# xiph/rav1e

Hardware: AMD Instinct MI355X
Metric: RDO-candidate Mpixels/s (dist+fwd_tx+mc) at 4K speed-6 (higher is better)
Workload: dtype u8

## Files before the change

rav1e_amd/csrc/cand_common.hpp:

```cpp
#pragma once
#include <type_traits>

#include "common.hpp"
#include "dist_common.hpp"
#include "mc_common.hpp"

namespace r1cand {

#include "mc_taps_packed.inc"

template <int CTRL>
__device__ __forceinline__ int32_t dpp(int32_t x) {
  return __builtin_amdgcn_update_dpp(0, x, CTRL, 0xf, 0xf, true);
}
template <int CTRL>
__device__ __forceinline__ int32_t bfly_lanes(int32_t x, int32_t sm) {
  return __mul24(x, sm | 1) + dpp<CTRL>(x);
}
struct LaneSigns { int32_t s1, s2; };
template <int TS>
__device__ __forceinline__ LaneSigns lane_signs(int lane) {
  LaneSigns s;
  if constexpr (TS == 8) {
    s.s1 = -(int32_t)((lane ^ (lane >> 2)) & 1);
    s.s2 = -(int32_t)(((lane >> 1) ^ (lane >> 2)) & 1);
  } else {
    s.s1 = -(int32_t)(lane & 1);
    s.s2 = 0;
  }
  return s;
}
template <int TS>
__device__ __forceinline__ uint32_t habs_lanes(int32_t x, LaneSigns sg) {
  x = bfly_lanes<0xB1>(x, sg.s1);
  if constexpr (TS == 8) x = bfly_lanes<0x4E>(x, sg.s2);
  const int32_t ax = iabs32(x);
  const int32_t ap = TS == 8 ? dpp<0x141>(ax) : dpp<0x4E>(ax);
  return (uint32_t)(ax > ap ? ax : ap);
}

__device__ __forceinline__ uint32_t sad_u32(uint32_t a, uint32_t b, uint32_t acc) {
  uint32_t r;
  asm("v_sad_u32 %0, %1, %2, %3" : "=v"(r) : "v"(a), "v"(b), "v"(acc));
  return r;
}

typedef short v2s_t __attribute__((ext_vector_type(2)));
typedef unsigned short v2us_t __attribute__((ext_vector_type(2)));
__device__ __forceinline__ uint32_t pk_add(uint32_t a, uint32_t b) {
  return __builtin_bit_cast(uint32_t, (v2s_t)(__builtin_bit_cast(v2s_t, a) + __builtin_bit_cast(v2s_t, b)));
}
__device__ __forceinline__ uint32_t pk_sub(uint32_t a, uint32_t b) {
  return __builtin_bit_cast(uint32_t, (v2s_t)(__builtin_bit_cast(v2s_t, a) - __builtin_bit_cast(v2s_t, b)));
}
__device__ __forceinline__ uint32_t pk_mad(uint32_t x, uint32_t s, uint32_t p) {
  uint32_t r;
  asm("v_pk_mad_i16 %0, %1, %2, %3" : "=v"(r) : "v"(x), "v"(s), "v"(p));
  return r;
}
__device__ __forceinline__ uint32_t pk_max(uint32_t a, uint32_t b) {
  uint32_t r;
  asm("v_pk_max_i16 %0, %1, %2" : "=v"(r) : "v"(a), "v"(b));
  return r;
}
__device__ __forceinline__ uint32_t pk_min(uint32_t a, uint32_t b) {
  uint32_t r;
  asm("v_pk_min_i16 %0, %1, %2" : "=v"(r) : "v"(a), "v"(b));
  return r;
}
__device__ __forceinline__ uint32_t pk_pair(int32_t lo, int32_t hi) {
  return __builtin_amdgcn_perm((uint32_t)hi, (uint32_t)lo, 0x05040100u);
}
__device__ __forceinline__ void pk_bfly8_s2(const uint32_t (&a)[8], uint32_t (&d)[8]) {
  uint32_t b[8];
#pragma unroll
  for (int k = 0; k < 4; k++) {
    b[2 * k] = pk_add(a[2 * k], a[2 * k + 1]);
    b[2 * k + 1] = pk_sub(a[2 * k], a[2 * k + 1]);
  }
  d[0] = pk_add(b[0], b[2]); d[2] = pk_sub(b[0], b[2]);
  d[1] = pk_add(b[1], b[3]); d[3] = pk_sub(b[1], b[3]);
  d[4] = pk_add(b[4], b[6]); d[6] = pk_sub(b[4], b[6]);
  d[5] = pk_add(b[5], b[7]); d[7] = pk_sub(b[5], b[7]);
}
__device__ __forceinline__ uint32_t habs_lanes_pk(uint32_t x, uint32_t m1, uint32_t m2, uint32_t acc) {
  x = pk_mad(x, m1, (uint32_t)dpp<0xB1>((int32_t)x));
  x = pk_mad(x, m2, (uint32_t)dpp<0x4E>((int32_t)x));
  const uint32_t ax = pk_max(x, pk_sub(0u, x));
  const uint32_t mx = pk_max(ax, (uint32_t)dpp<0x141>((int32_t)ax));
  return __builtin_amdgcn_udot2(__builtin_bit_cast(v2us_t, mx), __builtin_bit_cast(v2us_t, 0x00010001u),
                                acc, false);
}

__device__ __forceinline__ uint32_t ashr_pair(int32_t lo, int32_t hi, int sh) {
  return __builtin_amdgcn_perm((uint32_t)(hi >> sh), (uint32_t)(lo >> sh), 0x05040100u);
}

__device__ __forceinline__ int32_t dot2_seed0(uint32_t a, uint32_t b) {
  int32_t r;
  asm("v_dot2_i32_i16 %0, %1, %2, 0" : "=v"(r) : "v"(a), "v"(b));
  return r;
}
__device__ __forceinline__ int32_t dot2_seed64(uint32_t a, uint32_t b) {
  int32_t r;
  asm("v_dot2_i32_i16 %0, %1, %2, 64" : "=v"(r) : "v"(a), "v"(b));
  return r;
}
__device__ __forceinline__ int32_t dot2_seed(uint32_t a, uint32_t b, int32_t c_uniform) {
  int32_t r;
  asm("v_dot2_i32_i16 %0, %1, %2, %3" : "=v"(r) : "v"(a), "v"(b), "s"(c_uniform));
  return r;
}
__device__ __forceinline__ int32_t dot4_seed(uint32_t a, uint32_t b, int32_t c_uniform) {
  int32_t r;
  asm("v_dot4_i32_i8 %0, %1, %2, %3" : "=v"(r) : "v"(a), "v"(b), "s"(c_uniform));
  return r;
}

template <int BPP> struct Taps;
template <> struct Taps<1> { uint32_t fx0, fx1, ty[4]; };
template <> struct Taps<2> { uint32_t tx[4], ty[4]; };
template <int BPP, int W, int H>
__device__ __forceinline__ Taps<BPP> load_taps(int cf, int rf, int mx, int my) {
  const int fxi = r1mc::filter_index(mx, W), fyi = r1mc::filter_index(my, H);
  Taps<BPP> t;
  if constexpr (BPP == 1) {
    t.fx0 = kTapI8[fxi][cf][0];
    t.fx1 = kTapI8[fxi][cf][1];
  }
#pragma unroll
  for (int j = 0; j < 4; j++) {
    if constexpr (BPP == 2) t.tx[j] = kTapI16[fxi][cf][j];
    t.ty[j] = kTapI16[fyi][rf][j];
  }
  return t;
}
__device__ __forceinline__ bool taps_six(const Taps<1> &t) {
  return __all(((t.ty[0] & 0xffffu) | (t.ty[3] >> 16)) == 0);
}
__device__ __forceinline__ bool taps_six(const Taps<2> &t) {
  return __all(((t.ty[0] & 0xffffu) | (t.ty[3] >> 16) | (t.tx[0] & 0xffffu) | (t.tx[3] >> 16)) == 0);
}

#define R1_ODD_ROW_TAPS(ty, tz)                                                                   \
  do {                                                                                            \
    tz[0] = ty[0] << 16;                                                                          \
    _Pragma("unroll") for (int j = 1; j < 4; j++) tz[j] = __builtin_amdgcn_alignbit(ty[j], ty[j - 1], 16); \
    tz[4] = ty[3] >> 16;                                                                          \
  } while (0)

template <int W, int H, int WS, bool PREP, bool PACK4 = false>
__device__ __forceinline__ void mc8_column_t(const uint8_t *win, int c, const Taps<1> &tp, int32_t *pred, bool six) {
  const uint32_t fx0 = tp.fx0, fx1 = tp.fx1;
  uint32_t ty[4], tz[5];
#pragma unroll
  for (int j = 0; j < 4; j++) ty[j] = tp.ty[j];
  R1_ODD_ROW_TAPS(ty, tz);
  static_assert(!(PREP && PACK4), "the shift-free pack is stated for put_8tap only");
  constexpr int32_t bias = 8192 + 2 + (PREP ? 0 : 32);
  constexpr int WSD = WS / 4;
  const uint32_t *wrow = (const uint32_t *)win + (c >> 2);
  const uint32_t sh8 = 8u * (uint32_t)(c & 3);
  const uint64_t t64 = (((uint64_t)fx1 << 32) | fx0) << sh8;
  const uint32_t t0 = (uint32_t)t64, t1 = (uint32_t)(t64 >> 32);
  const uint32_t t2 = (uint32_t)(((uint64_t)fx1 << sh8) >> 32);
  auto hacc = [&](int r) -> int32_t {
    const uint32_t d0 = wrow[r * WSD], d1 = wrow[r * WSD + 1], d2 = wrow[r * WSD + 2];
    int32_t acc = dot4_seed(d0, t0, bias);
    acc = __builtin_amdgcn_sdot4((int)d1, (int)t1, acc, false);
    acc = __builtin_amdgcn_sdot4((int)d2, (int)t2, acc, false);
    return acc;
  };
  auto hpair = [&](int r) -> uint32_t {
    if constexpr (PACK4) {
      if (r + 1 < H + 7) return pk_pair(hacc(r), hacc(r + 1)) & 0xfffcfffcu;
      return (uint32_t)hacc(r) & 0xfffffffcu;
    } else {
      if (r + 1 < H + 7) return ashr_pair(hacc(r), hacc(r + 1), 2);
      return (uint32_t)(hacc(r) >> 2);
    }
  };
  auto body = [&](auto six_tag) {
    constexpr bool SIX = decltype(six_tag)::value;
    uint32_t pk[5];
    if constexpr (PACK4) pk[0] = SIX ? ((uint32_t)hacc(1) & 0xfffcu) << 16 : hpair(0);
    else pk[0] = SIX ? (uint32_t)(hacc(1) >> 2) << 16 : hpair(0);
#pragma unroll
    for (int j = 1; j < 4; j++) pk[j] = hpair(2 * j);
#pragma unroll
    for (int j = 0; j < H / 2; j++) {
      if (!SIX || j + 1 < H / 2) pk[4] = hpair(2 * j + 8);
      int32_t a0 = PREP ? dot2_seed64(pk[0], ty[0]) : dot2_seed0(pk[0], ty[0]);
#pragma unroll
      for (int k = 1; k < 4; k++)
        a0 = __builtin_amdgcn_sdot2(__builtin_bit_cast(v2s_t, pk[k]),
                                    __builtin_bit_cast(v2s_t, ty[k]), a0, false);
      int32_t a1;
      if constexpr (SIX) {
        a1 = PREP ? dot2_seed64(pk[1], tz[1]) : dot2_seed0(pk[1], tz[1]);
#pragma unroll
        for (int k = 2; k < 4; k++)
          a1 = __builtin_amdgcn_sdot2(__builtin_bit_cast(v2s_t, pk[k]),
                                      __builtin_bit_cast(v2s_t, tz[k]), a1, false);
      } else {
        a1 = PREP ? dot2_seed64(pk[0], tz[0]) : dot2_seed0(pk[0], tz[0]);
#pragma unroll
        for (int k = 1; k < 5; k++)
          a1 = __builtin_amdgcn_sdot2(__builtin_bit_cast(v2s_t, pk[k]),
                                      __builtin_bit_cast(v2s_t, tz[k]), a1, false);
      }
      if constexpr (PREP) {
        pred[2 * j] = a0 >> 7;
        pred[2 * j + 1] = a1 >> 7;
      } else {
        a0 >>= PACK4 ? 13 : 11;
        a1 >>= PACK4 ? 13 : 11;
        pred[2 * j] = a0 < 0 ? 0 : (a0 > 255 ? 255 : a0);
        pred[2 * j + 1] = a1 < 0 ? 0 : (a1 > 255 ? 255 : a1);
      }
#pragma unroll
      for (int k = 0; k < 4; k++) pk[k] = pk[k + 1];
    }
  };
  if (six) body(std::true_type{});
  else body(std::false_type{});
}

template <int W, int H, int WS, bool PREP>
__device__ __forceinline__ void mc16_column_t(const uint8_t *win, int c, const Taps<2> &tp, int bit_depth,
                                              int32_t *pred, bool six) {
  uint32_t tx[4], ty[4], tz[5];
#pragma unroll
  for (int j = 0; j < 4; j++) {
    tx[j] = tp.tx[j];
    ty[j] = tp.ty[j];
  }
  R1_ODD_ROW_TAPS(ty, tz);
  const int ib = r1mc::intermediate_bits(bit_depth);
  const int hsh = 7 - ib, vsh = 7 + ib;
  const int32_t hbias = (1 << (6 - ib)) + (PREP ? 0 : 64);
  const int32_t maxv = (1 << bit_depth) - 1;
  constexpr int WSD = WS / 4;
  const uint32_t *wrow = (const uint32_t *)win + (c >> 1);
  const bool odd = c & 1;
  uint32_t u[5];
  u[0] = odd ? tx[0] << 16 : tx[0];
#pragma unroll
  for (int j = 1; j < 4; j++) u[j] = odd ? __builtin_amdgcn_alignbit(tx[j], tx[j - 1], 16) : tx[j];
  u[4] = odd ? tx[3] >> 16 : 0u;
  auto body = [&](auto six_tag) {
    constexpr bool SIX = decltype(six_tag)::value;
    auto hacc = [&](int r) -> int32_t {
      const uint32_t *p = wrow + r * WSD;
      int32_t acc = dot2_seed(p[0], u[0], hbias);
#pragma unroll
      for (int j = 1; j < (SIX ? 4 : 5); j++)
        acc = __builtin_amdgcn_sdot2(__builtin_bit_cast(v2s_t, p[j]), __builtin_bit_cast(v2s_t, u[j]), acc, false);
      return acc;
    };
    auto hpair = [&](int r) -> uint32_t {
      if (r + 1 < H + 7) return ashr_pair(hacc(r), hacc(r + 1), hsh);
      return (uint32_t)(hacc(r) >> hsh);
    };
    uint32_t pk[5];
    pk[0] = SIX ? (uint32_t)(hacc(1) >> hsh) << 16 : hpair(0);
#pragma unroll
    for (int j = 1; j < 4; j++) pk[j] = hpair(2 * j);
#pragma unroll
    for (int j = 0; j < H / 2; j++) {
      if (!SIX || j + 1 < H / 2) pk[4] = hpair(2 * j + 8);
      int32_t a0 = PREP ? dot2_seed64(pk[0], ty[0]) : dot2_seed0(pk[0], ty[0]);
#pragma unroll
      for (int k = 1; k < 4; k++)
        a0 = __builtin_amdgcn_sdot2(__builtin_bit_cast(v2s_t, pk[k]), __builtin_bit_cast(v2s_t, ty[k]), a0, false);
      int32_t a1;
      if constexpr (SIX) {
        a1 = PREP ? dot2_seed64(pk[1], tz[1]) : dot2_seed0(pk[1], tz[1]);
#pragma unroll
        for (int k = 2; k < 4; k++)
          a1 = __builtin_amdgcn_sdot2(__builtin_bit_cast(v2s_t, pk[k]), __builtin_bit_cast(v2s_t, tz[k]), a1, false);
      } else {
        a1 = PREP ? dot2_seed64(pk[0], tz[0]) : dot2_seed0(pk[0], tz[0]);
#pragma unroll
        for (int k = 1; k < 5; k++)
          a1 = __builtin_amdgcn_sdot2(__builtin_bit_cast(v2s_t, pk[k]), __builtin_bit_cast(v2s_t, tz[k]), a1, false);
      }
      if constexpr (PREP) {
        pred[2 * j] = (a0 >> 7) - 8192;
        pred[2 * j + 1] = (a1 >> 7) - 8192;
      } else {
        a0 >>= vsh;
        a1 >>= vsh;
        pred[2 * j] = a0 < 0 ? 0 : (a0 > maxv ? maxv : a0);
        pred[2 * j + 1] = a1 < 0 ? 0 : (a1 > maxv ? maxv : a1);
      }
#pragma unroll
      for (int k = 0; k < 4; k++) pk[k] = pk[k + 1];
    }
  };
  if (six) body(std::true_type{});
  else body(std::false_type{});
}

template <int BPP, int W, int H, int WS, bool PREP, bool PACK4 = false>
__device__ __forceinline__ void mc_column_fast(const uint8_t *win, int c, const Taps<BPP> &tp, int bit_depth,
                                               int32_t *pred, bool six) {
  static_assert(!PACK4 || BPP == 1, "8 * mid of 16-bit pixels does not fit i16");
  if constexpr (BPP == 1) mc8_column_t<W, H, WS, PREP, PACK4>(win, c, tp, pred, six);
  else mc16_column_t<W, H, WS, PREP>(win, c, tp, bit_depth, pred, six);
}

__device__ __forceinline__ void satd_rows16_s2(const int32_t *v, uint32_t (&d)[8]) {
  uint32_t a[8];
#pragma unroll
  for (int k = 0; k < 8; k++) a[k] = pk_pair(v[k], v[8 + k]);
  pk_bfly8_s2(a, d);
}
template <int W, int H>
__device__ __forceinline__ void satd_tile_store(const int32_t *v, uint32_t *tcol) {
#pragma unroll
  for (int g = 0; g < H / 16; g++) {
    uint32_t d[8];
    satd_rows16_s2(v + g * 16, d);
#pragma unroll
    for (int k = 0; k < 4; k++) {
      tcol[(g * 8 + 2 * k) * W] = pk_add(d[k], d[k + 4]);
      tcol[(g * 8 + 2 * k + 1) * W] = pk_sub(d[k], d[k + 4]);
    }
  }
}
template <int NI, int P>
__device__ __forceinline__ uint32_t satd_tile_rows(const uint32_t *tile, int c) {
  uint32_t acc = 0;
#pragma unroll
  for (int m = 0; m < NI; m++) {
    const uint4 *p = (const uint4 *)(tile + (c + m * P) * 8);
    const uint4 lo = p[0], hi = p[1];
    const uint32_t x[8] = {lo.x, lo.y, lo.z, lo.w, hi.x, hi.y, hi.z, hi.w};
    uint32_t z[8];
    pk_bfly8_s2(x, z);
#pragma unroll
    for (int k = 0; k < 4; k++) {
      const uint32_t mx = pk_max(pk_max(z[k], z[k + 4]), pk_sub(0u, pk_min(z[k], z[k + 4])));
      acc = __builtin_amdgcn_udot2(__builtin_bit_cast(v2us_t, mx), __builtin_bit_cast(v2us_t, 0x00020002u), acc, false);
    }
  }
  return acc;
}

template <int TS, int H, int BD>
__device__ __forceinline__ uint32_t satd_column(const int32_t *v, int lane) {
  const LaneSigns sg = lane_signs<TS>(lane);
  uint32_t acc = 0;
  if constexpr (TS == 8 && BD <= 10) {
    const uint32_t m1 = (uint32_t)sg.s1 | 0x00010001u, m2 = (uint32_t)sg.s2 | 0x00010001u;
    if constexpr (H == 8) {
      uint32_t a[4];
#pragma unroll
      for (int k = 0; k < 4; k++) a[k] = pk_pair(v[k] + v[k + 4], v[k] - v[k + 4]);
      const uint32_t a0 = pk_add(a[0], a[1]), a1 = pk_sub(a[0], a[1]);
      const uint32_t a2 = pk_add(a[2], a[3]), a3 = pk_sub(a[2], a[3]);
      acc = habs_lanes_pk(pk_add(a0, a2), m1, m2, acc);
      acc = habs_lanes_pk(pk_add(a1, a3), m1, m2, acc);
      acc = habs_lanes_pk(pk_sub(a0, a2), m1, m2, acc);
      acc = habs_lanes_pk(pk_sub(a1, a3), m1, m2, acc);
    } else {
#pragma unroll
      for (int g = 0; g < H / 16; g++) {
        uint32_t d[8];
        satd_rows16_s2(v + g * 16, d);
#pragma unroll
        for (int k = 0; k < 4; k++) {
          acc = habs_lanes_pk(pk_add(d[k], d[k + 4]), m1, m2, acc);
          acc = habs_lanes_pk(pk_sub(d[k], d[k + 4]), m1, m2, acc);
        }
      }
    }
    return acc;
  }
#pragma unroll
  for (int g = 0; g < H / TS; g++) {
    int32_t a[TS];
#pragma unroll
    for (int k = 0; k < TS; k++) a[k] = v[g * TS + k];
    if constexpr (TS == 4) {
      const int32_t a0 = a[0] + a[1], a1 = a[0] - a[1];
      const int32_t a2 = a[2] + a[3], a3 = a[2] - a[3];
      a[0] = a0 + a2; a[1] = a1 + a3; a[2] = a0 - a2; a[3] = a1 - a3;
    } else {
      int32_t b[8], d[8];
#pragma unroll
      for (int k = 0; k < 4; k++) {
        b[2 * k] = a[2 * k] + a[2 * k + 1];
        b[2 * k + 1] = a[2 * k] - a[2 * k + 1];
      }
      d[0] = b[0] + b[2]; d[2] = b[0] - b[2];
      d[1] = b[1] + b[3]; d[3] = b[1] - b[3];
      d[4] = b[4] + b[6]; d[6] = b[4] - b[6];
      d[5] = b[5] + b[7]; d[7] = b[5] - b[7];
#pragma unroll
      for (int k = 0; k < 4; k++) {
        a[k] = d[k] + d[k + 4];
        a[k + 4] = d[k] - d[k + 4];
      }
    }
#pragma unroll
    for (int k = 0; k < TS; k++) acc += habs_lanes<TS>(a[k], sg);
  }
  return acc;
}

}
```

rav1e_amd/csrc/mc_window.hpp:

```cpp
#pragma once

namespace r1mc {

constexpr int window_stride(int w, int bpp) { return (((w + 7) * bpp + 3) >> 2) << 2; }

}
```

rav1e_amd/csrc/rdo_cand_kernel.hpp:

```cpp
#pragma once
#include <cstdlib>
#include <type_traits>

#include "cand_common.hpp"
#include "dist_common.hpp"
#include "intra_pred_common.hpp"
#include "itx_common.hpp"
#include "mc_common.hpp"
#include "quant_common.hpp"
#include "rdo_cand_args.hpp"
#include "tx_common.hpp"

#ifdef R1_PHASE_PROF
static __device__ unsigned long long g_phase[4096][8];
#define R1_PROF(i)                                                          \
  do {                                                                      \
    const unsigned long long t_ = __builtin_readcyclecounter();             \
    if (QM == 0 && threadIdx.x == 0 && (blockIdx.x & 63) == 0 && (blockIdx.x >> 6) < 4096) \
      g_phase[blockIdx.x >> 6][i] = t_ - tprev_;                            \
    tprev_ = t_;                                                            \
  } while (0)
#define R1_PROF_INIT unsigned long long tprev_ = __builtin_readcyclecounter()
#else
#define R1_PROF(i) do {} while (0)
#define R1_PROF_INIT do {} while (0)
#endif

namespace {
using r1tx::T;
using r1cand::sad_u32;

template <int BD, int WL, int HL, typename CT, int QM, bool MT = false, int PS = 0>
__global__ __launch_bounds__(64, rdo_waves_hint(BD, WL, HL, QM, MT)) void k_rdo_cand(
    R1Plane org, R1Plane ref, const R1RdoCand *__restrict__ cands, int n,
    uint32_t *__restrict__ sad_out, uint32_t *__restrict__ satd_out,
    CT *__restrict__ coeffs, void *__restrict__ pred_out, RdoQuantArgs qa,
    typename std::conditional<PS == 1, RdoIntraArgs, RdoNoIntraArgs>::type ia) {
  using PL = RdoCandPlan<BD, WL, HL, QM, MT, PS>;
  constexpr int BPP = PL::BPP, W = PL::W, H = PL::H, P = PL::P, NC = PL::NC, TS = PL::TS, WS = PL::WS, FL = PL::FL, HU = PL::HU;
  constexpr bool INTRA = PL::INTRA, SPLIT_T = PL::SPLIT_T, SRC_LDS = PL::SRC_LDS, SRC_LATE = PL::SRC_LATE,
                 SRC_KEEP = PL::SRC_KEEP, SATD_T = PL::SATD_T, COLSHARE = PL::COLSHARE;
  typedef typename PL::TB TB;
  constexpr int LSTRIDE = PL::LSTRIDE, ISTRIDE = PL::ISTRIDE, QT_STRIDE = PL::QT_STRIDE, SRC_ROW = PL::SRC_ROW,
                SRC_CSTRIDE = PL::SRC_CSTRIDE, SATD_STRIDE = PL::SATD_STRIDE, LDS_WORK = PL::LDS_WORK,
                SRC_OFF = PL::SRC_OFF, TKEEP_OFF = PL::TKEEP_OFF, LDS_BYTES = PL::LDS_BYTES;
  static_assert(!INTRA || LDS_BYTES <= RdoCandPlan<BD, WL, HL, QM, MT, 0>::LDS_BYTES,
                "an intra instantiation's LDS must not exceed its inter twin's");
  constexpr int SH0 = r1tx::fwd_shift_ct(WL, HL, BD, 0), SH1 = r1tx::fwd_shift_ct(WL, HL, BD, 1),
                SH2 = r1tx::fwd_shift_ct(WL, HL, BD, 2);
  constexpr bool COL_FOLD = PL::COL_FOLD;
  static_assert(!COL_FOLD || SH0 > 0, "the column family starts from a pending shift[0]");
  constexpr int SH1C = COL_FOLD ? 0 : SH1;
  constexpr bool HALVE2 = PL::HALVE2, MC_PACK4 = PL::MC_PACK4;
  __shared__ __attribute__((aligned(16))) uint8_t smem[LDS_BYTES];
  T *buf = (T *)smem;
  TB *tbuf = (TB *)smem;
  TB *tkeep = COLSHARE ? (TB *)(smem + TKEEP_OFF) : tbuf;

  R1_PROF_INIT;
  const unsigned wg = xcd_contiguous_wg();
  if ((long long)wg * NC >= (long long)n) return;
  const int lane = threadIdx.x;
  const int cl = lane / P, c = lane % P;
  const int cand_i = (int)wg * NC + cl;
  const long long cand = cand_i;
  constexpr bool UNMASK = !(BD == 8 && WL == 6 && HL == 6);
  const bool live_st = cand_i < n;
  const bool live = UNMASK || live_st;
  const int cl_ld = live_st ? cl : n - 1 - (int)wg * NC;
  const long long cand_ld = live_st ? cand : (long long)n - 1;
  R1RdoCand cd = {};
  R1IntraCand ic = {};
  int eset = 0;
  if constexpr (INTRA) {
    if (live) {
      ic = ia.cands[cand_ld];
      eset = (int)cand_ld / ia.edge_group;
      cd.ox = ia.pos_xy[2 * eset];
      cd.oy = ia.pos_xy[2 * eset + 1];
    }
  } else {
    if (live) cd = (cands + (size_t)wg * NC)[cl_ld];
  }
#ifdef R1_PHASE_PROF
  asm volatile("s_waitcnt vmcnt(0)" ::: "memory");
  R1_PROF(5);
#endif
  constexpr bool QUANT = QM != 0;
  constexpr int PPK = QM == 2 ? (H * BPP + 3) / 4 : 1;
  uint32_t ppk[PPK];
#pragma unroll
  for (int k = 0; k < PPK; k++) ppk[k] = 0;

  T v[H];
#pragma unroll
  for (int r = 0; r < H; r++) v[r] = 0;
  const bool col_live = live && c < W;
  const uint8_t *src_l = smem + SRC_OFF + cl * SRC_CSTRIDE + c * BPP;
  constexpr int CHS = SRC_ROW >= 16 ? 16 : SRC_ROW;
  constexpr int CPR = SRC_ROW / CHS;
  constexpr int RPP = P / CPR;
  constexpr int SPASS = SRC_LDS ? (H + RPP - 1) / RPP : 1;
  const int srow = c / CPR, sch = c - srow * CPR;
  U32x4 q[SPASS];
  if constexpr (SRC_LDS) {
    const uint8_t *po = (const uint8_t *)org.data +
                        (((uint32_t)(org.yorigin + cd.oy) * (uint32_t)org.stride + (uint32_t)(org.xorigin + cd.ox)) * BPP +
                         (uint32_t)(sch * CHS));
    const uint32_t so = (uint32_t)org.stride * BPP;
#pragma unroll
    for (int u = 0; u < SPASS; u++) {
      const int rr = srow + u * RPP;
      q[u] = U32x4{0, 0, 0, 0};
      if (live && rr < H) {
        if constexpr (CHS == 16) q[u] = ld_u32x4(po + rr * so);
        else if constexpr (CHS == 8) { const U32x2 t = ld_u32x2(po + rr * so); q[u].a = t.a; q[u].b = t.b; }
        else q[u].a = ld_u32(po + rr * so);
      }
    }
  } else if (col_live) {
    const uint8_t *po = px_addr<BPP>(org, cd.ox + c, cd.oy);
    const size_t so = (size_t)org.stride * BPP;
#pragma unroll
    for (int r = 0; r < H; r++) v[r] = ld_px<BPP>(po + r * so);
  }
  uint8_t *win = smem + cl * (H + 7) * WS;
  const bool from_ref = !INTRA && live && !qa.pred_in;
  r1mc::WindowStage<BPP, BPP == 1 ? 0x80808080u : 0u, W, H, P> wst;
  if (from_ref) wst.load(ref, cd.rx, cd.ry, c);
  r1cand::Taps<BPP> tp = {};
  if (from_ref) tp = r1cand::load_taps<BPP, W, H>(cd.col_frac, cd.row_frac, cd.mode_x, cd.mode_y);
  const bool six = r1cand::taps_six(tp);
  auto stage_source = [&]() {
    if (live) {
      uint8_t *sd = smem + SRC_OFF + cl * SRC_CSTRIDE + sch * CHS;
#pragma unroll
      for (int u = 0; u < SPASS; u++) {
        const int rr = srow + u * RPP;
        if (rr < H) {
          if constexpr (CHS == 16) *(uint4 *)(sd + rr * SRC_ROW) = make_uint4(q[u].a, q[u].b, q[u].c, q[u].d);
          else if constexpr (CHS == 8) *(uint2 *)(sd + rr * SRC_ROW) = make_uint2(q[u].a, q[u].b);
          else *(uint32_t *)(sd + rr * SRC_ROW) = q[u].a;
        }
      }
    }
  };
  if constexpr (SRC_LDS && !SRC_LATE && !INTRA) stage_source();
  if (from_ref) wst.store(win, WS);
  uint16_t *eraw = (uint16_t *)smem + cl * (5 * FL);
  int left_len = 0, above_len = 0;
  if constexpr (INTRA) {
    if (live) {
      left_len = ia.lens[2 * eset];
      above_len = ia.lens[2 * eset + 1];
      const uint8_t *e = (const uint8_t *)ia.edges + ((size_t)eset * ia.edge_stride + (2 * r1ip::MAXTX - (W + H))) * BPP;
      for (int k = c; k < FL; k += P) eraw[k] = (uint16_t)ld_px<BPP>(e + k * BPP);
    }
  }
#ifdef R1_PHASE_PROF
  asm volatile("s_waitcnt vmcnt(0)" ::: "memory");
  R1_PROF(6);
#endif
  __syncthreads();
  R1_PROF(0);

  uint32_t sad_acc = 0;
  if constexpr (INTRA) {
    const bool directional = live && r1ip::is_directional(ic.mode, ic.angle);
    const bool enable = directional && ic.ief != 0;
    const uint16_t *tl = eraw + (W + H);
    uint16_t *work = eraw + FL;
    int up_a = 0, up_l = 0;
    r1ip::edge_filter_upsample<const R1IntraCand &>(tl, 0, work, W, H, P, c, ic, enable, left_len, above_len,
                                                     (1 << BD) - 1, up_a, up_l);
    int32_t pred[H];
    if (col_live) {
      if (ic.mode == r1ip::UV_CFL_PRED && !ia.ac) ic.angle = 0;
      const int16_t *acb = ic.mode == r1ip::UV_CFL_PRED && ia.ac ? ia.ac + (size_t)cand_ld * (W * H) : nullptr;
      r1ip::predict_column<const R1IntraCand &>(W, H, c, ic, directional, enable, up_a, up_l, tl, 0, work, left_len, BD,
                                                 acb, [&](int i, int32_t pv) { pred[i] = pv; });
      if (pred_out && live_st) {
        if constexpr (BPP == 1) {
          uint8_t *pp = (uint8_t *)pred_out + (size_t)cand * W * H + c;
#pragma unroll
          for (int r = 0; r < H; r++) pp[(size_t)r * W] = (uint8_t)pred[r];
        } else {
          uint16_t *pp = (uint16_t *)pred_out + (size_t)cand * W * H + c;
#pragma unroll
          for (int r = 0; r < H; r++) pp[(size_t)r * W] = (uint16_t)pred[r];
        }
      }
      if constexpr (QM == 2) {
#pragma unroll
        for (int r = 0; r < H; r++) {
          if constexpr (BPP == 1) ppk[r >> 2] |= (uint32_t)pred[r] << (8 * (r & 3));
          else ppk[r >> 1] |= (uint32_t)pred[r] << (16 * (r & 1));
        }
      }
    }
    if constexpr (SRC_LDS) {
      __syncthreads();
      stage_source();
      __syncthreads();
    }
    if (col_live) {
      if constexpr (SRC_LDS) {
#pragma unroll
        for (int r = 0; r < H; r++) {
          const uint32_t sp = BPP == 1 ? (uint32_t)src_l[r * SRC_ROW] : (uint32_t) * (const uint16_t *)(src_l + r * SRC_ROW);
          sad_acc = sad_u32(sp, (uint32_t)pred[r], sad_acc);
          v[r] = (T)sp - pred[r];
        }
      } else {
#pragma unroll
        for (int r = 0; r < H; r++) v[r] -= pred[r];
      }
    }
  } else
  if constexpr (BPP == 1) {
    if (col_live) {
      int32_t pred[H];
      if (qa.pred_in) {
        const uint8_t *pi = (const uint8_t *)qa.pred_in + (size_t)cand_ld * W * H + c;
#pragma unroll
        for (int r = 0; r < H; r++) pred[r] = pi[(size_t)r * W];
      } else {
        r1cand::mc_column_fast<BPP, W, H, WS, false, MC_PACK4>(win, c, tp, BD, pred, six);
      }
      if (pred_out && live_st) {
        uint8_t *pp = (uint8_t *)pred_out + (size_t)cand * W * H + c;
#pragma unroll
        for (int r = 0; r < H; r++) pp[(size_t)r * W] = (uint8_t)pred[r];
      }
      if constexpr (QM == 2) {
#pragma unroll
        for (int r = 0; r < H; r++) ppk[r >> 2] |= (uint32_t)pred[r] << (8 * (r & 3));
      }
      if constexpr (SRC_LDS) {
#pragma unroll
        for (int r = 0; r < H; r++) {
          const uint32_t sp = src_l[r * SRC_ROW];
          sad_acc = sad_u32(sp, (uint32_t)pred[r], sad_acc);
          v[r] = (T)sp - pred[r];
        }
      } else {
#pragma unroll
        for (int r = 0; r < H; r++) v[r] -= pred[r];
      }
    }
  } else {
    int32_t pred[H];
    if (col_live) {
      if (qa.pred_in) {
        const uint16_t *pi = (const uint16_t *)qa.pred_in + (size_t)cand_ld * W * H + c;
#pragma unroll
        for (int r = 0; r < H; r++) pred[r] = pi[(size_t)r * W];
      } else {
        r1cand::mc_column_fast<BPP, W, H, WS, false>(win, c, tp, BD, pred, six);
      }
      if (pred_out && live_st) {
        uint16_t *pp = (uint16_t *)pred_out + (size_t)cand * W * H + c;
#pragma unroll
        for (int r = 0; r < H; r++) pp[(size_t)r * W] = (uint16_t)pred[r];
      }
      if constexpr (QM == 2) {
#pragma unroll
        for (int r = 0; r < H; r++) ppk[r >> 1] |= (uint32_t)pred[r] << (16 * (r & 1));
      }
    }
    if constexpr (SRC_LATE) {
      __syncthreads();
      stage_source();
      __syncthreads();
    }
    if (col_live) {
      if constexpr (SRC_LDS) {
#pragma unroll
        for (int r = 0; r < H; r++) {
          const uint32_t sp = *(const uint16_t *)(src_l + r * SRC_ROW);
          sad_acc = sad_u32(sp, (uint32_t)pred[r], sad_acc);
          v[r] = (T)sp - pred[r];
        }
      } else {
#pragma unroll
        for (int r = 0; r < H; r++) v[r] -= pred[r];
      }
    }
  }
  R1_PROF(1);
  if (sad_out) {
    uint32_t sad = sad_acc;
    if constexpr (!SRC_LDS) {
#pragma unroll
      for (int r = 0; r < H; r++) sad += (uint32_t)iabs32(v[r]);
    }
    const uint32_t s = group_sum<P>(sad);
    if (live_st && c == 0) (sad_out + (size_t)wg * NC)[cl] = s;
  }
  if (satd_out) {
    uint32_t part;
    if constexpr (SATD_T) {
      uint32_t *tile = (uint32_t *)smem + cl * SATD_STRIDE;
      __syncthreads();
      if (c < W) r1cand::satd_tile_store<W, H>(v, tile + c);
      __syncthreads();
      part = r1cand::satd_tile_rows<(W < H ? W : H) / 16, P>(tile, c);
    } else {
      part = r1cand::satd_column<TS, H, BD>(v, lane);
    }
    const uint32_t s = group_sum<P>(part);
    constexpr int LN = TS == 4 ? 2 : 3;
    if (live_st && c == 0) (satd_out + (size_t)wg * NC)[cl] = (s + ((1u << LN) >> 1)) >> LN;
  }
  R1_PROF(2);
  if (!QUANT && !coeffs) return;

  constexpr bool MT_RECOMP = MT && SRC_KEEP;
  T vkeep[MT && !MT_RECOMP ? H : 1];
  if constexpr (MT && !MT_RECOMP) {
#pragma unroll
    for (int r = 0; r < H; r++) vkeep[r] = v[r];
  }
  constexpr bool TAIL_DEFER = MT && QM == 2 && W == 8 && H == 8;
  const bool tail_defer = TAIL_DEFER && qa.dist_kind == R1_DIST_CDEF && qa.nt <= 8;
  r1dist::CdefMoments tail_keep;
  uint32_t rem = MT ? qa.tx_mask : 1u;
  bool fresh = true;
  do {
  int t0 = 0;
  uint32_t gmask = 1u;
  if constexpr (MT) {
    t0 = (int)__builtin_ctz(rem);
    gmask = 1u << t0;
    if constexpr (COLSHARE) {
      auto colkey = [](int t) { return r1tx::vtx_1d(t) | ((int)r1tx::ud_flip(t) << 4) | ((int)r1tx::lr_flip(t) << 5); };
      const int k0 = colkey(t0);
      for (uint32_t m = rem & (rem - 1); m != 0; m &= m - 1) {
        const int t = (int)__builtin_ctz(m);
        if (colkey(t) == k0) gmask |= 1u << t;
      }
    }
    rem &= ~gmask;
    if (!fresh) {
      if constexpr (MT_RECOMP) {
        if (col_live) {
#pragma unroll
          for (int r = 0; r < H; r++) {
            const T sp = BPP == 1 ? (T)src_l[r * SRC_ROW] : (T) * (const uint16_t *)(src_l + r * SRC_ROW);
            const T pr = BPP == 1 ? (T)((ppk[r >> 2] >> (8 * (r & 3))) & 0xFF)
                                  : (T)((ppk[r >> 1] >> (16 * (r & 1))) & 0xFFFF);
            v[r] = sp - pr;
          }
        }
      } else {
#pragma unroll
        for (int r = 0; r < H; r++) v[r] = vkeep[r];
      }
    }
    fresh = false;
  }
  __syncthreads();
  const int tx_col = MT ? t0 : (QM != 0 && qa.tx_mask != 0 ? (int)__builtin_ctz(qa.tx_mask) : (int)cd.tx_type);
  constexpr bool TX_VOTE = rdo_tx_vote(WL, HL, QM, MT, PS);
  static_assert(!TX_VOTE || UNMASK, "the vote reads every lane's descriptor");
  int tx_s = 0;
  bool tx_uni = false, col_uni = false, row_uni = false;
  if constexpr (TX_VOTE) {
    tx_s = __builtin_amdgcn_readfirstlane(tx_col);
    tx_uni = __all(tx_col == tx_s);
    col_uni = tx_uni && r1tx::vtx_1d(tx_s) != 3;
    row_uni = tx_uni && r1tx::htx_1d(tx_s) != 3;
  }
  bool any_ud;
  if (TX_VOTE && tx_uni) any_ud = r1tx::ud_flip(tx_s);
  else any_ud = __any(live && r1tx::ud_flip(tx_col));
  if (col_live) {
    if (any_ud) {
      const bool ud = r1tx::ud_flip(tx_col);
#pragma unroll
      for (int r = 0; r < H / 2; r++) {
        const T t0 = v[r], t1 = v[H - 1 - r];
        v[r] = ud ? t1 : t0;
        v[H - 1 - r] = ud ? t0 : t1;
      }
    }
    if constexpr (COL_FOLD) {
      if (TX_VOTE && col_uni) r1tx::fwd_col_m24_kernel<H, SH0, SH1, HALVE2>(v, r1tx::vtx_1d(tx_s));
      else r1tx::fwd_col_m24<H, SH0, SH1, HALVE2>(v, r1tx::vtx_1d(tx_col));
    } else {
#pragma unroll
      for (int r = 0; r < H; r++) v[r] = r1tx::shift_fwd_ct<SH0>(v[r]);
      if (TX_VOTE && col_uni) r1tx::fwd_1d_m24_kernel<H, HALVE2>(v, r1tx::vtx_1d(tx_s));
      else r1tx::fwd_1d_m24<H, HALVE2>(v, r1tx::vtx_1d(tx_col));
    }
    if constexpr (!SPLIT_T) {
      const int cc = cl * W + (r1tx::lr_flip(tx_col) ? W - 1 - c : c);
#pragma unroll
      for (int r = 0; r < HU; r++)
        tkeep[r * LSTRIDE + cc] = (TB)r1tx::shift_fwd_ct<SH1C>(v[r]);
    }
  }
  if constexpr (!SPLIT_T) __syncthreads();
  R1_PROF(3);
  do {
  const int tx_type = MT ? (int)__builtin_ctz(gmask) : tx_col;
  const int slot = MT ? (int)__builtin_popcount(qa.tx_mask & ((1u << tx_type) - 1u)) : 0;
  const long long oslot = MT ? cand * (long long)qa.nt + slot
                             : (QM != 0 && qa.nt != 0 ? cand * (long long)qa.nt + qa.slot : cand);
  const int cl2 = cl, r = c;
  const bool live2 = live;
  const bool row_live = live2 && r < HU;
  const int tt = tx_type;
  constexpr int OS = H < 32 ? H : 32, WC = W < 32 ? W : 32;
  T u[W];
  if constexpr (SPLIT_T) {
    const int cc = r1tx::lr_flip(tx_type) ? W - 1 - c : c;
#pragma unroll
    for (int half = 0; half < HU / 32; half++) {
      if (col_live) {
#pragma unroll
        for (int rr = 0; rr < 32; rr++)
          tbuf[rr * LSTRIDE + cc] = (TB)r1tx::shift_fwd_ct<SH1C>(v[half * 32 + rr]);
      }
      __syncthreads();
      if (row_live && (r >> 5) == half) {
#pragma unroll
        for (int k = 0; k < W; k++) u[k] = tbuf[(r & 31) * LSTRIDE + k];
      }
      __syncthreads();
    }
  }
  if (row_live) {
    if constexpr (!SPLIT_T) {
#pragma unroll
      for (int k = 0; k < W; k++) u[k] = tkeep[r * LSTRIDE + cl2 * W + k];
    }
    if (TX_VOTE && row_uni) r1tx::fwd_1d_m24_kernel<W, HALVE2>(u, r1tx::htx_1d(tx_s));
    else r1tx::fwd_1d_m24<W, HALVE2>(u, r1tx::htx_1d(tt));
#pragma unroll
    for (int k = 0; k < W; k++) {
      u[k] = r1tx::shift_fwd_ct<SH2>(u[k]);
      if constexpr (QUANT) u[k] = (T)(CT)u[k];
    }
  }
  if constexpr (MT) {
  } else
  if constexpr (P > 16) {
    if (coeffs && row_live && live_st) {
      CT *dst = coeffs + (size_t)wg * (NC * W * H) + (cl2 * (W * H) + (r >= 32 ? OS * WC : 0) + (r & 31));
#pragma unroll
      for (int cg = 0; cg < W; cg += 32)
#pragma unroll
        for (int k = 0; k < WC; k++) __builtin_nontemporal_store((CT)u[k + cg], &dst[H * cg + k * OS]);
    }
  } else
  if (coeffs) {
    constexpr int ESZ = (int)sizeof(CT);
    constexpr int NP = NC * W * H * ESZ > LDS_WORK ? 2 : 1;
    static_assert(NP == 1 || W == 64, "only the 64-wide blocks are split");
    static_assert(NC * W * H * ESZ / NP <= LDS_WORK, "a pass fits the LDS of the kernel");
    constexpr int EPP = W * H / NP;
    constexpr int CBY = EPP * ESZ;
    constexpr int CH = CBY / P >= 16 ? 16 : CBY / P;
    constexpr int NCH = CBY / P / CH;
    static_assert(CH * NCH * P == CBY && (CH == 16 || CH == 8 || CH == 4), "whole chunks");
    constexpr int TPAD = NC > 1 ? ((P * ESZ + 15) & ~15) / ESZ : 0;
    static_assert(NC * (EPP + TPAD) * ESZ <= LDS_WORK, "the padded tiles fit the LDS of the kernel");
    static_assert(((EPP + TPAD) * ESZ) % 16 == 0, "16-byte reads stay aligned");
    CT *tile = (CT *)smem + cl2 * (EPP + TPAD);
    uint8_t *gdst = (uint8_t *)(coeffs + (size_t)wg * (NC * W * H)) + cl2 * (W * H * ESZ);
#pragma unroll
    for (int p = 0; p < NP; p++) {
      __syncthreads();
      if (row_live) {
        constexpr int KP = W / NP;
#pragma unroll
        for (int k = p * KP; k < (p + 1) * KP; k++) {
          const int e = (r >= 32 ? OS * WC : 0) + (r & 31) + H * (k & ~31) + (k & 31) * OS - p * EPP;
          tile[e] = (CT)u[k];
        }
      }
      __syncthreads();
      if (live_st) {
        const uint8_t *src = (const uint8_t *)tile + r * CH;
        uint8_t *dst = gdst + p * CBY + r * CH;
#pragma unroll
        for (int j = 0; j < NCH; j++) {
          if constexpr (CH == 16) {
            typedef uint32_t u32x4_t __attribute__((ext_vector_type(4)));
            __builtin_nontemporal_store(*(const u32x4_t *)(src + j * P * CH), (u32x4_t *)(dst + j * P * CH));
          } else if constexpr (CH == 8) {
            typedef uint32_t u32x2_t __attribute__((ext_vector_type(2)));
            __builtin_nontemporal_store(*(const u32x2_t *)(src + j * P * CH), (u32x2_t *)(dst + j * P * CH));
          } else {
            __builtin_nontemporal_store(*(const uint32_t *)(src + j * P * CH), (uint32_t *)(dst + j * P * CH));
          }
        }
      }
    }
  }
  R1_PROF(4);
  if constexpr (QUANT) {
    constexpr int CODED = OS * WC;
    constexpr int PL = WL > HL ? WL : HL;
    constexpr int NPLQ = CODED / P;
    static_assert(CODED % P == 0 && NPLQ >= 1, "P lanes share the coded area");
    __syncthreads();
    int32_t *tile = (int32_t *)smem + cl2 * QT_STRIDE;
    unsigned long long tail = 0;
    if (row_live) {
#pragma unroll
      for (int k = 0; k < W; k++) {
        if (r < 32 && k < 32) {
          tile[k * OS + r] = u[k];
        } else {
          tail += (unsigned long long)(long long)(int32_t)((uint32_t)u[k] * (uint32_t)u[k]);
        }
      }
    }
    __syncthreads();
    const int kind = tt < 10 ? 0 : ((tt & 1) ? 2 : 1);
    int eob = 0;
    unsigned long long dist = 0;
    constexpr int LTS = (W * H > 256) + (W * H > 1024);
#ifndef R1_QUANT_MID
#define R1_QUANT_MID 0
#endif
    constexpr bool QMID = R1_QUANT_MID && sizeof(CT) == 4;
    r1q::quantize_group<CT, PL, NPLQ, QM == 1, LTS, QMID>(tile, cl2 * P, r, live2, qa.scan[kind], qa.qp, tail,
// ... 230 lines not shown
```

rav1e_amd/csrc/rdo_cand_plan.hpp:

```cpp
#pragma once
#include <cstdint>
#include <type_traits>

#include "mc_window.hpp"

constexpr int rdo_waves_hint(int bd, int wl, int hl, int qm, bool mt = false) {
  if (mt) {
    if (wl <= 3 && hl <= 3) return qm == 2 ? (bd == 8 ? 7 : 6) : 1;
    return qm == 2 ? 4 : 1;
  }
  if (wl == 5 && hl == 5 && qm == 0 && bd != 8) return 6;
  if (wl == 3 && hl == 3 && qm == 2) return 8;
  if (wl == 4 && hl == 4 && qm == 2) return bd == 8 ? 6 : 5;
  if (wl == 5 && hl == 5 && qm == 2) return 4;
  if (wl == 5 && hl == 5 && qm == 1) return 5;
  if (wl == 6 && hl == 6 && qm == 2) return bd == 8 ? 4 : 3;
  return 1;
}

constexpr bool rdo_tx_size_exists(int wl, int hl) {
  return wl >= 2 && wl <= 6 && hl >= 2 && hl <= 6 && wl - hl <= 2 && hl - wl <= 2;
}
constexpr bool rdo_type_fanout(int wl, int hl) { return wl <= 4 && hl <= 4; }
constexpr bool r1_intra_two_launch(int wl, int hl, int bd, int qm) {
  return wl == hl && ((wl == 4 && (qm == 1 || bd != 8)) || (wl == 6 && qm == 1 && bd != 8) ||
                      (wl == 5 && qm == 2 && bd != 8));
}
enum RdoIntraRoute { RDO_INTRA_FANOUT, RDO_INTRA_PER_TYPE, RDO_INTRA_TWO_LAUNCH };
constexpr RdoIntraRoute rdo_intra_route(int wl, int hl, int bd, int qm) {
  return r1_intra_two_launch(wl, hl, bd, qm) ? RDO_INTRA_TWO_LAUNCH
                                             : (rdo_type_fanout(wl, hl) ? RDO_INTRA_FANOUT : RDO_INTRA_PER_TYPE);
}
constexpr bool rdo_cand_instantiated(int bd, int wl, int hl, int qm, bool mt, int ps) {
  if (!(bd == 8 || bd == 10 || bd == 12) || !rdo_tx_size_exists(wl, hl) || qm < 0 || qm > 2 || ps < 0 || ps > 1)
    return false;
  if (ps == 1)
    return qm != 0 && rdo_intra_route(wl, hl, bd, qm) == (mt ? RDO_INTRA_FANOUT : RDO_INTRA_PER_TYPE);
  return !mt || (qm != 0 && rdo_type_fanout(wl, hl));
}

constexpr bool rdo_tx_vote(int wl, int hl, int qm, bool mt, int ps) {
  return qm == 0 && !mt && ps == 0 && wl <= 4 && hl <= 4;
}

constexpr bool rdo_col_fold(int bd, int wl, int hl, int qm, bool mt, int ps) {
  if (mt || ps != 0 || wl != hl) return false;
  if (bd == 8) return qm == 0 ? (wl >= 3 && wl <= 5) : (qm == 1 && (wl == 3 || wl == 4));
  return bd == 10 && qm == 0 && (wl == 4 || wl == 5);
}

constexpr bool rdo_plain_square(int wl, int hl, int qm, bool mt, int ps) {
  return qm == 0 && !mt && ps == 0 && wl == hl && wl >= 3 && wl <= 6;
}
constexpr bool rdo_halve2(int bd, int wl, int hl, int qm, bool mt, int ps) {
  if (!rdo_plain_square(wl, hl, qm, mt, ps)) return false;
  return bd == 8 || (bd == 10 && (wl == 4 || wl == 6));
}
constexpr bool rdo_mc_pack4(int bd, int wl, int hl, int qm, bool mt, int ps) {
  return bd == 8 && rdo_plain_square(wl, hl, qm, mt, ps) && wl <= 5;
}

template <int BD, int WL, int HL, int QM, bool MT, int PS>
struct RdoCandPlan {
  static constexpr int BPP = BD == 8 ? 1 : 2;
  static constexpr bool INTRA = PS == 1;
  static constexpr int W = 1 << WL, H = 1 << HL;
  static constexpr int P = W > H ? W : H, NC = 64 / P;
  static constexpr int TS = (W < H ? W : H) == 4 ? 4 : 8;
  static constexpr bool COL_FOLD = rdo_col_fold(BD, WL, HL, QM, MT, PS);
  static constexpr bool HALVE2 = rdo_halve2(BD, WL, HL, QM, MT, PS);
  static constexpr bool MC_PACK4 = rdo_mc_pack4(BD, WL, HL, QM, MT, PS);
  static constexpr int WS = r1mc::window_stride(W, BPP);
  static constexpr int WIN_BYTES = INTRA ? 0 : NC * (H + 7) * WS;
  static constexpr int FL = 2 * (W + H) + 1;
  static constexpr int EDGE_BYTES = INTRA ? ((NC * 5 * FL * 2 + 15) & ~15) : 0;
  static constexpr bool TB16 = (BD == 10 && WL == 5 && HL == 5) || (MT && W <= 16 && H <= 16);
  typedef typename std::conditional<TB16, int16_t, int32_t>::type TB;
  static constexpr int LSTRIDE = NC * W + (TB16 ? 2 : 1);
  static constexpr int ISTRIDE = NC * W + 1;
  static constexpr bool SPLIT_T = W == 64 && H == 64;
  static constexpr int TXB_ROWS = SPLIT_T ? 32 : H;
  static constexpr int TXB_BYTES = TXB_ROWS * LSTRIDE * (int)sizeof(TB);
  static constexpr int IRB_BYTES = QM == 2 ? (H < 32 ? H : 32) * ISTRIDE * 4 : 0;
  static constexpr int QT_PAD = NC > 2 ? P : 0;
  static constexpr int QT_STRIDE = (W < 32 ? W : 32) * (H < 32 ? H : 32) + QT_PAD;
  static constexpr int QT_BYTES = QM != 0 ? NC * QT_STRIDE * 4 : 0;
  static constexpr int HU = (QM == 2 && H > 32) ? 32 : H;
  static constexpr int REC_BYTES = QM == 2 ? NC * W * H * BPP : 0;
  static constexpr bool SRC_LDS = BPP == 1 || P <= 32;
  static constexpr bool SRC_LATE0 = SRC_LDS && BD != 8 && (P == 32 || (P == 16 && QM == 0));
  static constexpr int SRC_ROW = W * BPP;
  static constexpr int WIN_PAD = (WIN_BYTES + 15) & ~15;
  static constexpr int SRC_CSTRIDE = H * SRC_ROW + (NC > 1 ? (SRC_ROW > 16 ? SRC_ROW : 16) : 0);
  static constexpr int SRC_BYTES = SRC_LDS ? NC * SRC_CSTRIDE : 0;
  static constexpr bool SRC_KEEP = QM == 2 && H <= 16 && SRC_LDS && !SRC_LATE0;
  static constexpr bool SRC_LATE = INTRA ? SRC_LDS && !SRC_KEEP : SRC_LATE0;
  static constexpr int WS_BYTES =
      SRC_KEEP ? WIN_PAD : (SRC_LATE ? (WIN_PAD > SRC_BYTES ? WIN_PAD : SRC_BYTES) : WIN_PAD + SRC_BYTES);
  static constexpr int LDS_A0 = WS_BYTES > TXB_BYTES ? WS_BYTES : TXB_BYTES;
  static constexpr int LDS_A = LDS_A0 > IRB_BYTES ? LDS_A0 : IRB_BYTES;
  static constexpr int SATD_STRIDE = W * H / 2 + (NC > 1 ? P : 0);
  static constexpr int SATD_BYTES = NC * SATD_STRIDE * 4;
  static constexpr bool SATD_T = TS == 8 && BD <= 10 && (W < H ? W : H) >= 16 && SATD_BYTES <= LDS_A &&
                                 !(QM == 2 && WL == 6 && HL == 6);
  static_assert(SATD_STRIDE % 4 == 0, "16-byte reads stay aligned");
  static constexpr int LDS_B = QT_BYTES > REC_BYTES ? QT_BYTES : REC_BYTES;
  static constexpr int LDS_WORK = ((LDS_A > LDS_B ? LDS_A : LDS_B) + 15) & ~15;
  static constexpr int SRC_OFF = SRC_KEEP ? LDS_WORK : (SRC_LATE ? 0 : WIN_PAD);
  static constexpr bool COLSHARE = MT && !SPLIT_T;
  static constexpr int TKEEP_OFF = (LDS_WORK + (SRC_KEEP ? SRC_BYTES : 0) + 15) & ~15;
  static constexpr int LDS_CHAIN =
      COLSHARE ? TKEEP_OFF + H * LSTRIDE * (int)sizeof(TB) : LDS_WORK + (SRC_KEEP ? SRC_BYTES : 0);
  static constexpr int LDS_BYTES = LDS_CHAIN > EDGE_BYTES ? LDS_CHAIN : EDGE_BYTES;
};
```

Baseline: 679,400.

## Compute 8-bit MC horizontal filter with MFMA i8 matrix ops for 32x32/64x64

For 8-bit plain square blocks of 32x32 and 64x64, the horizontal subpel filter pass now uses mfma_i32_16x16x32_i8 instead of per-lane sdot4 dot products. Each lane loads 8-byte fragments of the MC window as the A operand, and a banded tap matrix is built per lane from wave-uniform taps read with readlane. One MFMA yields four rows at once. For two candidates per wave, a zeroed LDS shadow region masks the other candidate's fragment. The aim is to move filter arithmetic onto matrix cores, at the cost of the zeroing stores, extra LDS space and the assumption that taps are uniform across each candidate's lanes.

```diff
diff --git a/rav1e_amd/csrc/cand_common.hpp b/rav1e_amd/csrc/cand_common.hpp
--- a/rav1e_amd/csrc/cand_common.hpp
+++ b/rav1e_amd/csrc/cand_common.hpp
@@ -149,8 +149,10 @@
     tz[4] = ty[3] >> 16;                                                                          \
   } while (0)
 
-template <int W, int H, int WS, bool PREP, bool PACK4 = false>
-__device__ __forceinline__ void mc8_column_t(const uint8_t *win, int c, const Taps<1> &tp, int32_t *pred, bool six) {
+typedef int v4i_t __attribute__((ext_vector_type(4)));
+template <int W, int H, int WS, bool PREP, bool PACK4 = false, int MXNC = 0>
+__device__ __forceinline__ void mc8_column_t(const uint8_t *win, int c, const Taps<1> &tp, int32_t *pred, bool six,
+                                             int lane = 0, const uint8_t *zero = nullptr) {
   const uint32_t fx0 = tp.fx0, fx1 = tp.fx1;
   uint32_t ty[4], tz[5];
 #pragma unroll
@@ -164,7 +166,33 @@
   const uint64_t t64 = (((uint64_t)fx1 << 32) | fx0) << sh8;
   const uint32_t t0 = (uint32_t)t64, t1 = (uint32_t)(t64 >> 32);
   const uint32_t t2 = (uint32_t)(((uint64_t)fx1 << sh8) >> 32);
+  static_assert(MXNC == 0 || ((MXNC == 1 || MXNC == 2) && W == 64 / MXNC && WS % 8 == 0), "matrix pass: 64x64, 32x32");
+  const uint8_t *ap0 = win, *ap1 = win;
+  long bb0 = 0, bb1 = 0;
+  if constexpr (MXNC != 0) {
+    const uint8_t *ad = win + r1mc::mx_a_offset(lane, MXNC, H, WS);
+    const bool second = MXNC == 2 && r1mc::mx_a_cand(lane, MXNC) == 1;
+    ap0 = second ? zero : ad;
+    ap1 = second ? ad : zero;
+    bb0 = (long)r1mc::mx_band8((uint32_t)__builtin_amdgcn_readlane((int)fx0, 0),
+                               (uint32_t)__builtin_amdgcn_readlane((int)fx1, 0), lane);
+    if constexpr (MXNC == 2)
+      bb1 = (long)r1mc::mx_band8((uint32_t)__builtin_amdgcn_readlane((int)fx0, 32),
+                                 (uint32_t)__builtin_amdgcn_readlane((int)fx1, 32), lane);
+  }
+  const v4i_t cbias = {bias, bias, bias, bias};
+  v4i_t quad = cbias;
+  int quad_at = -1;
   auto hacc = [&](int r) -> int32_t {
+    if constexpr (MXNC != 0) {
+      if ((r >> 2) != quad_at) {
+        quad_at = r >> 2;
+        quad = __builtin_amdgcn_mfma_i32_16x16x32_i8(*(const long *)(ap0 + quad_at * 4 * WS), bb0, cbias, 0, 0, 0);
+        if constexpr (MXNC == 2)
+          quad = __builtin_amdgcn_mfma_i32_16x16x32_i8(*(const long *)(ap1 + quad_at * 4 * WS), bb1, quad, 0, 0, 0);
+      }
+      return quad[r & 3];
+    }
     const uint32_t d0 = wrow[r * WSD], d1 = wrow[r * WSD + 1], d2 = wrow[r * WSD + 2];
     int32_t acc = dot4_seed(d0, t0, bias);
     acc = __builtin_amdgcn_sdot4((int)d1, (int)t1, acc, false);
@@ -302,11 +330,12 @@
   else body(std::false_type{});
 }
 
-template <int BPP, int W, int H, int WS, bool PREP, bool PACK4 = false>
+template <int BPP, int W, int H, int WS, bool PREP, bool PACK4 = false, int MXNC = 0>
 __device__ __forceinline__ void mc_column_fast(const uint8_t *win, int c, const Taps<BPP> &tp, int bit_depth,
-                                               int32_t *pred, bool six) {
+                                               int32_t *pred, bool six, int lane = 0, const uint8_t *zero = nullptr) {
   static_assert(!PACK4 || BPP == 1, "8 * mid of 16-bit pixels does not fit i16");
-  if constexpr (BPP == 1) mc8_column_t<W, H, WS, PREP, PACK4>(win, c, tp, pred, six);
+  static_assert(MXNC == 0 || BPP == 1, "there is no i16 matrix type");
+  if constexpr (BPP == 1) mc8_column_t<W, H, WS, PREP, PACK4, MXNC>(win, c, tp, pred, six, lane, zero);
   else mc16_column_t<W, H, WS, PREP>(win, c, tp, bit_depth, pred, six);
 }
 
diff --git a/rav1e_amd/csrc/mc_window.hpp b/rav1e_amd/csrc/mc_window.hpp
--- a/rav1e_amd/csrc/mc_window.hpp
+++ b/rav1e_amd/csrc/mc_window.hpp
@@ -4,4 +4,20 @@
 
 constexpr int window_stride(int w, int bpp) { return (((w + 7) * bpp + 3) >> 2) << 2; }
 
+constexpr int mx_a_offset(int l, int nc, int h, int ws) {
+  const int m = l & 15, g = m >> 2, k = m & 3, gpc = 4 / nc;
+  return (g / gpc) * (h + 7) * ws + k * ws + 16 * (g % gpc) + 8 * (l >> 4);
 }
+constexpr int mx_a_cand(int l, int nc) { return ((l & 15) >> 2) / (4 / nc); }
+constexpr int mx_quads(int h) { return (h + 7 + 3) / 4; }
+constexpr int mx_a_end(int nc, int h, int ws) {
+  return mx_a_offset(63, nc, h, ws) + (mx_quads(h) - 1) * 4 * ws + 8;
+}
+constexpr int mx_zero_bytes(int h, int ws) { return (((mx_quads(h) - 1) * 4 * ws + 8) + 15) & ~15; }
+constexpr unsigned long long mx_band8(unsigned fx0, unsigned fx1, int l) {
+  const unsigned long long t = ((unsigned long long)fx1 << 32) | fx0;
+  const int d = (l & 15) - 8 * (l >> 4);
+  return d >= 8 || d <= -8 ? 0ull : (d >= 0 ? t << (8 * d) : t >> (8 * -d));
+}
+
+}
diff --git a/rav1e_amd/csrc/rdo_cand_kernel.hpp b/rav1e_amd/csrc/rdo_cand_kernel.hpp
--- a/rav1e_amd/csrc/rdo_cand_kernel.hpp
+++ b/rav1e_amd/csrc/rdo_cand_kernel.hpp
@@ -52,6 +52,9 @@
   static_assert(!COL_FOLD || SH0 > 0, "the column family starts from a pending shift[0]");
   constexpr int SH1C = COL_FOLD ? 0 : SH1;
   constexpr bool HALVE2 = PL::HALVE2, MC_PACK4 = PL::MC_PACK4;
+  constexpr int MX_NC = PL::MX_NC;
+  static_assert(MX_NC == 0 || (BPP == 1 && QM == 0 && !INTRA && P == W && NC * W == 64),
+                "a coefficient kernel of 8-bit pixels, lane = (candidate, column) with no idle lane");
   __shared__ __attribute__((aligned(16))) uint8_t smem[LDS_BYTES];
   T *buf = (T *)smem;
   TB *tbuf = (TB *)smem;
@@ -131,6 +134,12 @@
   r1cand::Taps<BPP> tp = {};
   if (from_ref) tp = r1cand::load_taps<BPP, W, H>(cd.col_frac, cd.row_frac, cd.mode_x, cd.mode_y);
   const bool six = r1cand::taps_six(tp);
+  if constexpr (PL::MX_ZERO_BYTES != 0) {
+#pragma unroll
+    for (int k = 0; k < (PL::MX_ZERO_BYTES / 16 + 63) / 64; k++)
+      if (lane + 64 * k < PL::MX_ZERO_BYTES / 16)
+        *(uint4 *)(smem + PL::MX_ZERO_OFF + 16 * (lane + 64 * k)) = make_uint4(0u, 0u, 0u, 0u);
+  }
   auto stage_source = [&]() {
     if (live) {
       uint8_t *sd = smem + SRC_OFF + cl * SRC_CSTRIDE + sch * CHS;
@@ -225,6 +234,10 @@
 #pragma unroll
         for (int r = 0; r < H; r++) pred[r] = pi[(size_t)r * W];
       } else {
+        if constexpr (MX_NC != 0)
+          r1cand::mc_column_fast<BPP, W, H, WS, false, MC_PACK4, MX_NC>(smem, c, tp, BD, pred, six, lane,
+                                                                         smem + PL::MX_ZERO_OFF);
+        else
         r1cand::mc_column_fast<BPP, W, H, WS, false, MC_PACK4>(win, c, tp, BD, pred, six);
       }
       if (pred_out && live_st) {
diff --git a/rav1e_amd/csrc/rdo_cand_plan.hpp b/rav1e_amd/csrc/rdo_cand_plan.hpp
--- a/rav1e_amd/csrc/rdo_cand_plan.hpp
+++ b/rav1e_amd/csrc/rdo_cand_plan.hpp
@@ -59,6 +59,9 @@
 constexpr bool rdo_mc_pack4(int bd, int wl, int hl, int qm, bool mt, int ps) {
   return bd == 8 && rdo_plain_square(wl, hl, qm, mt, ps) && wl <= 5;
 }
+constexpr bool rdo_mc_matrix(int bd, int wl, int hl, int qm, bool mt, int ps) {
+  return bd == 8 && rdo_plain_square(wl, hl, qm, mt, ps) && wl >= 5;
+}
 
 template <int BD, int WL, int HL, int QM, bool MT, int PS>
 struct RdoCandPlan {
@@ -112,4 +115,13 @@
   static constexpr int LDS_CHAIN =
       COLSHARE ? TKEEP_OFF + H * LSTRIDE * (int)sizeof(TB) : LDS_WORK + (SRC_KEEP ? SRC_BYTES : 0);
   static constexpr int LDS_BYTES = LDS_CHAIN > EDGE_BYTES ? LDS_CHAIN : EDGE_BYTES;
+  static constexpr bool MC_MATRIX = rdo_mc_matrix(BD, WL, HL, QM, MT, PS);
+  static constexpr int MX_NC = MC_MATRIX ? NC : 0;
+  static constexpr int MX_ZERO_BYTES = MC_MATRIX && NC > 1 ? r1mc::mx_zero_bytes(H, WS) : 0;
+  static constexpr int MX_ZERO_OFF = (WIN_PAD + SRC_BYTES + 15) & ~15;
+  static_assert(!MC_MATRIX || (NC <= 2 && WS % 8 == 0 && !SRC_LATE && !SRC_KEEP && SRC_OFF == WIN_PAD),
+                "the matrix pass reads aligned 8-byte fragments of one or two windows; the shadow follows the source");
+  static_assert(!MC_MATRIX || r1mc::mx_a_end(NC > 2 ? 2 : NC, H, WS) <= LDS_BYTES,
+                "the furthest byte an A fragment reads lies inside the allocation");
+  static_assert(!MC_MATRIX || MX_ZERO_OFF + MX_ZERO_BYTES <= LDS_BYTES, "the zeroed shadow lies inside the allocation");
 };
```

Measured after the change: 702,900, median of 6. 1.03x the previous value.
